# balazs-bamer/cdpr-simulation

Hardware: AMD Instinct MI355X
Metric: CDPR sim-steps/sec (whole node), 65 536 parallel 8-cable robots, 1 ms dt (higher is better)
Workload: dtype f32

## Files before the change

cdpr-simulation_amd/csrc/cdpr_engine.hip:

```cpp
#include "cdpr_engine_internal.hpp"

namespace {
thread_local std::string g_create_error;
}


namespace cdpr_host {

int derivative_weights(uint32_t n, uint32_t degree, double* w) {
  if (n < 2 || n > CDPR_MAX_D_BUFFER || degree < 1 || degree > CDPR_MAX_D_DEGREE || degree >= n) return CDPR_ERR_INVALID;
  const int m = (int)degree + 1;
  long double a[5][10];
  for (int i = 0; i < m; ++i)
    for (int j = 0; j < 2 * m; ++j) a[i][j] = 0.0L;
  std::vector<long double> x(n);
  for (uint32_t j = 0; j < n; ++j) x[j] = (long double)j - (long double)(n - 1) / 2.0L;
  for (int i = 0; i < m; ++i) {
    for (int k = 0; k < m; ++k) {
      long double s = 0;
      for (uint32_t j = 0; j < n; ++j) s += powl(x[j], i + k);
      a[i][k] = s;
    }
    a[i][m + i] = 1.0L;
  }
// ... 274 lines not shown
    case KernelId::PhysStep: return pick_phys_kernel(n, h->plan.fk, h->plan.td, kPhysStep);
    case KernelId::Rollout: return pick_rollout_kernel(n, h->plan.fk, h->plan.td);
    case KernelId::PhysRollout: return pick_phys_kernel(n, h->plan.fk, h->plan.td, kPhysRollout);
    case KernelId::PrSingle: return pick_pr_kernel(true, false, false, n, h->plan.fk, h->plan.td);
    case KernelId::PrLowreg: return pick_pr_kernel(true, false, true, n, h->plan.fk, h->plan.td);
    case KernelId::PrSplit: return pick_pr_split_kernel(n);
    case KernelId::PrMulti: return pick_pr_kernel(false, false, false, n, h->plan.fk, h->plan.td);
    case KernelId::PrRollout: return pick_pr_kernel(false, true, false, n, h->plan.fk, h->plan.td);
    case KernelId::PairSingle: return pick_pair_kernel(true, n, h->plan.fk, h->plan.td);
    case KernelId::PairMulti: return pick_pair_kernel(false, n, h->plan.fk, h->plan.td);
    case KernelId::PairStream: return pick_pair_stream_kernel(n, h->mode == kModeVelocity);
    case KernelId::Cable: return pick_cable_kernel(n, h->plan.fk, h->plan.td);
    default: return nullptr;
  }
}
StepKernel select_step_kernel(const cdpr_engine* h, int k, bool steady) { return step_kernel_of(h, planned_kernel(h->plan, launch_shape(h, k, steady))); }
bool pair_stream_steady(const cdpr_engine* h, const StepArgs& a) {
  return h->step != 0 && h->mode != kModeForce && a.pid_calls >= a.nbuf && h->cfg.publish_period == 0.0 && !a.dbg && !a.travel_on &&
         !(a.vel_limit > 0.f) && !a.unilateral && a.effort >= 0.f && a.clamp_cmd && !h->sched_ready;
}
bool split_steady_launch(const cdpr_engine* h, const PlannedKernel& pk, const StepArgs& a) {
  return pk.id == KernelId::Split && h->split_steady && !h->plan.per_robot && h->step != 0 && h->mode != kModeForce && a.pid_calls != 0 &&
         a.pid_calls >= a.nbuf && h->cfg.publish_period == 0.0 && !a.dbg && !a.travel_on;
}
uint32_t step_block_threads(const cdpr_engine* h, int k) { return planned_kernel(h->plan, launch_shape(h, k)).block; }

static int build_general(cdpr_engine* h) {
  const cdpr_config_t& cfg = h->cfg;
  h->glay.n = (int)h->n;
  h->glay.nb = (int)std::max(cfg.velocity_pid.d_buffer_length, cfg.position_pid.d_buffer_length);
  h->glay.ncas = (int)std::max(std::max(cfg.velocity_pid.p_filter.cascade, cfg.velocity_pid.d_filter.cascade),
                               std::max(cfg.position_pid.p_filter.cascade, cfg.position_pid.d_filter.cascade));
  const size_t rec_bytes = h->glay.bytes(h->stride);
  if (rec_bytes >= (1ull << 32)) {
    h->err = "general controller path: the controller records of this batch pass 4 GiB; split the batch over several handles";
    return CDPR_ERR_UNSUPPORTED;
  }
  CREATE_TRY(h, "hipMalloc(rec)", h->d_rec.alloc(rec_bytes));
  fill_gen_pid(cfg.position_pid, h->gpid[0]);
  fill_gen_pid(cfg.velocity_pid, h->gpid[1]);
  const int nbmax = h->glay.nb > 11 ? kGenMaxBuf : 11, nbp = gen_nbp(nbmax);
  std::vector<float> wt((size_t)2 * nbmax * nbp, 0.f);
  const cdpr_pid_params_t* pp[2] = {&cfg.position_pid, &cfg.velocity_pid};
  float w_new[2] = {0.f, 0.f};
  for (int p = 0; p < 2; ++p) {
    double w[CDPR_MAX_D_BUFFER];
// ... 99 lines not shown
  StepArgs a = h->base;
  a.state = st.as<float4>();
  a.obs = ob.as<float4>();
  a.cmd = cm.as<float>();
  a.dbg = nullptr;
  a.geom = h->d_geom;
  a.batch = h->plan.lane_cable ? (h->n <= 4 ? 16u : 8u) : h->plan.lane_pair ? 32u : 64u;
  a.stride = rows;
  a.nsteps = 1;
  a.obs_step_stride = 0;
  a.flags = 0u;
  a.publish_mask = 1ull;
  copy_pid(h->plan.per_robot ? h->pid_vel : h->pid_pos, a);
  copy_pid_alt(h->pid_pos, a.alt);
  a.meta = mt.as<uint8_t>();
  a.pid_calls = kCallSat;
  a.ring_slot = 0;
  set_weight_row(h, a);
  hipLaunchKernelGGL(select_step_kernel(h, 1), dim3(1), dim3(step_block_threads(h, 1)), 0, h->stream, a);
  HIP_TRY(h, hipGetLastError());
  if (planned_kernel(h->plan, launch_shape(h, 1)).id == KernelId::Split && h->split_steady) {
    for (const bool vel : {false, true}) {
      copy_pid(vel ? h->pid_vel : h->pid_pos, a);
      hipLaunchKernelGGL(pick_split_steady_kernel(h->n, vel), dim3(1), dim3(128), 0, h->stream, a);
      HIP_TRY(h, hipGetLastError());
    }
  }
  HIP_TRY(h, wait_stream(h));
  return CDPR_OK;
}

void launch_step(cdpr_engine* h, StepKernel kern, uint32_t robots_per_block, dim3 block, const StepArgs& a, uint32_t max_grid = 0) {
  const uint32_t B = a.batch;
  const uint32_t chunk = (h->plan.chunk && B > h->plan.chunk) ? h->plan.chunk : B;
  const uint32_t pieces = (B + chunk - 1u) / chunk;
  const uint32_t each = (((B + pieces - 1u) / pieces) + 63u) & ~63u;
  for (uint32_t first = 0; first < B; first += each) {
    StepArgs c = a;
    c.batch = std::min(each, B - first);
    c.state = a.state + first;
    c.obs = a.obs + first;
    if (a.cmd) c.cmd = a.cmd + (size_t)first * h->n;
    if (a.dbg) c.dbg = a.dbg + (size_t)first * CDPR_PID_DEBUG_AXES;
    if (a.meta) c.meta = a.meta + first;
    uint32_t grid = (c.batch + robots_per_block - 1u) / robots_per_block;
    if (max_grid && grid > max_grid) grid = max_grid;
    hipLaunchKernelGGL(kern, dim3(grid), block, 0, h->stream, c);
// ... 156 lines not shown
    a.cmd = h->d_target;
    a.meta = h->d_mode;
  } else {
    copy_pid(h->mode == kModeVelocity ? h->pid_vel : h->pid_pos, a);
    a.cmd = h->cmd[cmd_kind_of_mode(h->mode)].latched();
  }
  const uint32_t robots_per_block = h->plan.lane_cable ? (h->n <= 4 ? 16u : 8u) : h->plan.lane_pair ? 32u : 64u;
  const dim3 grid((h->batch + robots_per_block - 1u) / robots_per_block);

  constexpr int kGraphChunk = 10;
  int done = 0;
  while (done < nsteps) {
    const int k = std::min(per_launch, nsteps - done);
    a.nsteps = k;
    a.flags = h->plan.per_robot ? 0u : (h->mode == kModeVelocity ? kFlagActualIsVelocity : h->mode == kModeForce ? kFlagForceMode : 0u);
    const bool first_world = (h->step == 0);
    if (first_world) a.flags |= kFlagFirstWorldStep;
    a.pid_calls = sat_pid_calls(h->pid_calls);
    a.ring_slot = ring_slot_of(h->step);
    set_weight_row(h, a);
    const int kk = h->sched_refresh ? std::max(k, 2) : k;
    const PlannedKernel pk = planned_kernel(h->plan, launch_shape(h, kk, pair_stream_steady(h, a)));
    StepKernel kern = step_kernel_of(h, pk);
    h->last_variant = split_steady_launch(h, pk, a) ? 1 : 0;
    if (h->last_variant) kern = pick_split_steady_kernel(h->n, h->mode == kModeVelocity);
    const dim3 block(pk.block);
    const bool stream = pk.id == KernelId::PairStream;
    auto weights_for = [&](StepArgs& x) {
      const int slot = x.ring_slot;
      if (stream) x.ring_slot = 0;
      set_weight_row(h, x);
      x.ring_slot = slot;
    };
    if (stream) weights_for(a);
    h->last_kernel = pk;

    if (record) a.obs = record + (size_t)done * image;
    const bool steady = !record && !h->sched_refresh && h->use_graphs && (size_t)h->batch * h->n <= 131072u && !first_world && (h->plan.per_robot || a.pid_calls == kCallSat || h->mode == kModeForce) &&
                        h->cfg.publish_period == 0.0 && (nsteps - done) >= kGraphChunk * k;
    if (steady) {
      a.publish_mask = (k >= 64) ? ~0ull : ((1ull << k) - 1ull);
      cdpr_engine::GraphEntry* ge = nullptr;
      for (auto& g : h->graphs)
        if (g.kern == (void*)kern && g.cmd == a.cmd && g.steps_per_launch == k && g.flags == a.flags && g.start_slot == a.ring_slot) ge = &g;
      if (!ge) {
        cdpr_engine::GraphEntry g{(void*)kern, a.cmd, k, kGraphChunk, a.ring_slot, a.flags, nullptr, nullptr};
        bool captured = hipStreamBeginCapture(h->stream, hipStreamCaptureModeThreadLocal) == hipSuccess;
        if (captured) {
// ... 126 lines not shown
int checked(cdpr_engine* h, int rc) { return rc != CDPR_OK ? rc : check_fault(h); }

static int build_handle(cdpr_engine* h) {
  const cdpr_config_t& cfg = h->cfg;
  h->n = cfg.n_cables;
  h->batch = (uint32_t)cfg.batch;
  h->stride = (h->batch + 63u) & ~63u;
  if (h->stride % 131072u == 0u) h->stride += 128u;
  if (const char* sp = std::getenv("CDPR_STRIDE_PAD")) h->stride = ((h->batch + 63u) & ~63u) + ((uint32_t)(std::max(0L, std::atol(sp)) + 63L) & ~63u);
  h->dbg = (cfg.stages & CDPR_STAGE_PID_DEBUG) != 0;
  if (h->plan.persist) {
    h->persist_grid = (uint32_t)h->cus * 4u;
    if (const char* pg = std::getenv("CDPR_PERSIST_GRID")) h->persist_grid = (uint32_t)std::max(1L, std::atol(pg));
  }
  h->n_state = h->plan.general ? plat_slots(h->plan.fk) : state_slots((int)h->n, h->plan.fk);
  h->n_obs = obs_slots((int)h->n);
  memset(&h->base, 0, sizeof h->base);
  fill_consts(cfg, h->base);
  fill_pid(cfg.velocity_pid, cfg.dt, h->pid_vel, h->wtab_host[0]);
  fill_pid(cfg.position_pid, cfg.dt, h->pid_pos, h->wtab_host[1]);
  engine_reset_host(h);
  {
    if (const char* ss = std::getenv("CDPR_SPLIT_STEADY")) h->split_steady = !(ss[0] == '0');
    const char* ng = std::getenv("CDPR_NO_GRAPH");
    h->use_graphs = !(ng && ng[0] == '1');
  }

  CREATE_TRY(h, "hipSetDevice", hipSetDevice(h->device));
  CREATE_TRY(h, "hipStreamCreate", hipStreamCreateWithFlags(&h->stream, hipStreamNonBlocking));
  CREATE_TRY(h, "hipEventCreate", hipEventCreate(&h->ev0));
  CREATE_TRY(h, "hipEventCreate", hipEventCreate(&h->ev1));
  if (h->plan.fp64) {
    if (int rc = build_f64(h)) return rc;
  } else {
    const size_t slot_bytes = (size_t)h->stride * sizeof(float4);
    CREATE_TRY(h, "hipMalloc(state)", h->d_state.alloc(slot_bytes * h->n_state));
    CREATE_TRY(h, "hipMalloc(obs)", h->d_obs.alloc(slot_bytes * h->n_obs));
  }
  const size_t cmd_bytes = (size_t)h->stride * h->n * sizeof(float);
  for (int i = 0; i < 2; ++i)
    for (CmdChannel& c : h->cmd) {
      CREATE_TRY(h, "hipMalloc(cmd)", c.d[i].alloc(cmd_bytes));
      (void)hipMemset(c.d[i], 0, cmd_bytes);
    }
  if (int rc = upload_table(h, h->d_wtab, h->wtab_host, sizeof h->wtab_host, "wtab")) return rc;
  h->pid_vel.wtab = h->d_wtab;
// ... 610 lines not shown
  if (!h->plan.td) {
    h->err = "CDPR_STAGE_TD not enabled";
    return CDPR_ERR_UNSUPPORTED;
  }
  int rc = cdpr_get_joint_states(h, nullptr, nullptr, tension);
  if (rc != CDPR_OK) return rc;
  rc = h->plan.fp64 ? fetch_int_row64(h, kF64ObsFlags, infeasible) : fetch_fields(h, h->d_obs, {{3, 3}}, infeasible, 1u);
  if (rc == CDPR_OK && infeasible)
    for (uint32_t b = 0; b < h->batch; ++b) infeasible[b] &= 1;
  return checked(h, rc);
}

int cdpr_get_limit_state(cdpr_handle_t h, uint32_t* cable_mask) {
  if (!h || !cable_mask) return CDPR_ERR_INVALID;
  if (set_device(h) != CDPR_OK) return CDPR_ERR_DEVICE;
  int rc = h->plan.fp64 ? fetch_int_row64(h, kF64ObsFlags, reinterpret_cast<int32_t*>(cable_mask)) : fetch_fields(h, h->d_obs, {{3, 3}}, cable_mask, 1u);
  if (rc == CDPR_OK)
    for (uint32_t b = 0; b < h->batch; ++b) cable_mask[b] >>= 1;
  return checked(h, rc);
}

int cdpr_debug_last_variant(cdpr_handle_t h) { return h ? h->last_variant : -1; }

#ifdef CDPR_STAMPS
int cdpr_debug_set_stamps(cdpr_handle_t h, unsigned long long* d_stamps) {
  if (!h) return CDPR_ERR_INVALID;
  h->base.stamps = d_stamps;
  return CDPR_OK;
}
#endif

int cdpr_device_malloc(cdpr_handle_t h, size_t bytes, void** out) {
  if (!h || !out) return CDPR_ERR_INVALID;
  if (set_device(h) != CDPR_OK) return CDPR_ERR_DEVICE;
  HIP_TRY(h, hipMalloc(out, bytes));
  return CDPR_OK;
}

int cdpr_device_free(cdpr_handle_t h, void* ptr) {
  if (!h) return CDPR_ERR_INVALID;
  if (set_device(h) != CDPR_OK) return CDPR_ERR_DEVICE;
  HIP_TRY(h, hipFree(ptr));
  return CDPR_OK;
}

int cdpr_device_upload(cdpr_handle_t h, void* dst, const void* src, size_t bytes) {
// ... 37 lines not shown
```

cdpr-simulation_amd/csrc/cdpr_engine_internal.hpp:

```cpp
#pragma once
#include <hip/hip_runtime.h>

#include <atomic>
#include <chrono>

#include <algorithm>
#include <cmath>
#include <cstdio>
#include <cstring>
#include <cstdlib>
#include <string>
#include <vector>

#include "../../include/cdpr.h"
#include "cdpr_kernels.hpp"
#include "cdpr_select.hpp"
#include "cdpr_latch.hpp"
#include "cdpr_solvers.hpp"

using namespace cdpr;

namespace cdpr_host {

enum Mode { kModeForce = 0, kModePosition = 1, kModeVelocity = 2 };
// ... 118 lines not shown
  DevBuf<float> d_rec;
  DevBuf<float> d_gwtab;
  DevBuf<float> d_gptab;
  GenPid gpid[2]{};
  GenLayout glay{};
  DevBuf<double> d_roll64, d_roll64_acc;
  DevBuf<float> d_roll64_cmd;
  DevBuf<uint8_t> d_roll64_meta;
  size_t roll64_cols = 0;
  DevBuf<float> d_roll_rec;
  size_t roll_rec_cols = 0;
  struct GraphEntry {
    void* kern;
    const float* cmd;
    int steps_per_launch, launches, start_slot;
    uint32_t flags;
    hipGraph_t graph;
    hipGraphExec_t exec;
  };
  std::vector<GraphEntry> graphs;
  PlannedKernel last_kernel;
  int last_variant = 0;
  bool split_steady = true;
  int cus = 256;
  bool use_graphs = true;
  CmdChannel cmd[kCmdKinds];
  DevBuf<uint8_t> d_mode;
  DevBuf<float> d_target;
  hipStream_t copy_stream = nullptr;
  int mode = kModePosition;
  uint64_t step = 0;
  double prev_publish = 0.0;
  StepArgs base{};
  StepArgs pid_vel{}, pid_pos{};
  DevBuf<float> d_wtab;
  float wtab_host[2][kWin * (kWin + 2)]{};
  hipEvent_t ev0 = nullptr, ev1 = nullptr;
  uint64_t launches = 0, launches_mark = 0;
  PinnedBuf<float> h_pub;
  PinnedBuf<uint64_t> h_pub_done;
  DevBuf<uint32_t> d_pub_arrivals;
  uint64_t pub_epoch = 0;
  DevBuf<float> d_roll_ref;
  DevBuf<float> d_roll_cost;
  uint64_t roll_pending = 0;
  DevBuf<char> d_reset_args;
// ... 126 lines not shown
```

cdpr-simulation_amd/csrc/cdpr_kernels.hpp:

```cpp
#pragma once
#include "cdpr_step_kernel.hpp"
#include "cdpr_step_kernel_f64.hpp"
#include "cdpr_general_step.hpp"

namespace cdpr {

using StepKernel = void (*)(const StepArgs);
using F64Kernel = void (*)(const F64Args);
using GenKernel = void (*)(const StepArgs, const GenCtl);

#define CDPR_PICK_STAGES(N, EXPR)                 \
  do {                                            \
    if constexpr ((N) >= 6) {                     \
      if (fk && td) return EXPR(N, true, true);   \
      if (fk) return EXPR(N, true, false);        \
      if (td) return EXPR(N, false, true);        \
    }                                             \
    return EXPR(N, false, false);                 \
  } while (0)
#define CDPR_PICK_CABLES(FN, ...)          \
  switch (n) {                             \
    case 1: return FN<1>(__VA_ARGS__);     \
    case 2: return FN<2>(__VA_ARGS__);     \
    case 3: return FN<3>(__VA_ARGS__);     \
// ... 3 lines not shown
    case 7: return FN<7>(__VA_ARGS__);     \
    case 8: return FN<8>(__VA_ARGS__);     \
  }                                        \
  return nullptr

#define CDPR_PICK_CABLES12(FN, ...)        \
  switch (n) {                             \
    case 9: return FN<9>(__VA_ARGS__);     \
    case 10: return FN<10>(__VA_ARGS__);   \
    case 11: return FN<11>(__VA_ARGS__);   \
    case 12: return FN<12>(__VA_ARGS__);   \
  }                                        \
  CDPR_PICK_CABLES(FN, __VA_ARGS__)

StepKernel pick_step_kernel(bool single, uint32_t n, bool fk, bool td);
StepKernel pick_lowreg_kernel(uint32_t n, bool td);
StepKernel pick_rollout_kernel(uint32_t n, bool fk, bool td);
enum PhysKind { kPhysStep, kPhysRollout };
StepKernel pick_phys_kernel(uint32_t n, bool fk, bool td, int kind);
StepKernel pick_pr_kernel(bool single, bool rollout, bool lowreg, uint32_t n, bool fk, bool td);
StepKernel pick_onestep_kernel(uint32_t n, bool fk, bool td);
StepKernel pick_onestep_persist_kernel(uint32_t n, bool fk, bool td);
StepKernel pick_split_kernel(uint32_t n);
StepKernel pick_split_steady_kernel(uint32_t n, bool vel);
StepKernel pick_pr_split_kernel(uint32_t n);
StepKernel pick_pair_kernel(bool single, uint32_t n, bool fk, bool td);
StepKernel pick_pair_stream_kernel(uint32_t n, bool vel);
StepKernel pick_cable_kernel(uint32_t n, bool fk, bool td);
GenKernel pick_gen_kernel(uint32_t n, bool fk, bool td, bool rollout, bool long_window, bool single);
GenKernel pick_gen_lean11(uint32_t n);
GenKernel pick_gen_split11(uint32_t n);
F64Kernel pick_f64_split_kernel(uint32_t n, bool lean);
F64Kernel pick_f64_hold_pr_kernel(uint32_t n, bool full);
F64Kernel pick_f64_hold_long_kernel(uint32_t n, bool pr, bool tstop);
F64Kernel pick_f64_tstop_kernel(uint32_t n, bool pr = false, int hold = 0);
F64Kernel pick_f64_long_kernel(uint32_t n, bool pr = false, bool tstop = false);
F64Kernel pick_f64_split_hold_kernel(uint32_t n, bool lean, bool full);
F64Kernel pick_f64_pr_kernel(uint32_t n, bool ring_lds);
F64Kernel pick_f64_hold_kernel(uint32_t n, bool full);
F64Kernel pick_f64_kernel(uint32_t n, bool ring_lds, bool jcache);

}
```

cdpr-simulation_amd/csrc/cdpr_onestep_kernel.hpp:

```cpp
#pragma once
#include "cdpr_step_kernel.hpp"

namespace cdpr {

CDPR_DEV void row_to_lds(const float4* src, float4* dst_row) {
  __builtin_amdgcn_global_load_lds((const __attribute__((address_space(1))) void*)src, (__attribute__((address_space(3))) void*)dst_row, 16, 0, 0);
}


template <int NP, bool PR = false, bool FULL = false>
CDPR_DEV void pid_pairs(const StepArgs& a, int calls, bool is_vel, const v2f (&desired)[NP], const v2f (&actual)[NP], const v2f (&win)[NP][kWin],
                        v2f (&ierr)[NP], v2f (&f)[NP], v2f (&e_new)[NP], float& dbg_p, float& dbg_i, float& dbg_d, bool is_force = false) {
  const PidCoef c = pid_coef<PR>(a, is_vel);
  const bool run = (!PR || calls != 0) && !is_force;
  const bool full = FULL || calls >= c.nbuf;
  const float (&wt)[kWin + 2] = a.wrow;
  v2f error[NP], acc[NP];
#pragma unroll
  for (int k = 0; k < NP; ++k) {
    error[k] = desired[k] - actual[k];
    acc[k] = splat(wt[kWin]) * error[k];
  }
#pragma unroll
  for (int j = 0; j < kWin; ++j) {
// ... 364 lines not shown
  p3 = make_float4(n3.x, n3.y, n3.z, n3.w), p4 = make_float4(n4.x, n4.y, n4.z, n4.w);
  staged = run_pid;
  }
}

#ifndef CDPR_CTL_LOAD_DELAY
#define CDPR_CTL_LOAD_DELAY 8
#endif
#ifndef CDPR_SPLIT_PRIO
#define CDPR_SPLIT_PRIO 1
#endif
#ifdef CDPR_STAMPS
#define CDPR_SPLIT_STAMP(i)                                                                                          \
  do {                                                                                                               \
    __builtin_amdgcn_sched_barrier(0);                                                                               \
    if (a.stamps && lane == 0) a.stamps[(size_t)blockIdx.x * 8 + (i)] = __builtin_amdgcn_s_memrealtime();           \
    __builtin_amdgcn_sched_barrier(0);                                                                               \
  } while (0)
#else
#define CDPR_SPLIT_STAMP(i) do { } while (0)
#endif
#if defined(CDPR_STAMPS) && defined(CDPR_STAMPS_ITER)
#define CDPR_CTL_STAMP(i) do { } while (0)
#else
#define CDPR_CTL_STAMP(i) CDPR_SPLIT_STAMP(i)
#endif

template <int N, int XS, int ES, bool RAISED = true>
CDPR_DEV void split_estimator_wave(const StepArgs& a, float* geo, float gval, uint32_t lane, bool live, size_t st, uint32_t off, uint32_t woff,
                                   const float4& p0, const float4& p1, const float4& p3, const v2f* x_force, v2f* x_tension, float* x_est) {
  constexpr int NP = cable_pairs(N);
#if defined(CDPR_STAMPS) && defined(CDPR_STAMPS_CLOCK)
  const unsigned long long clk0 = __builtin_amdgcn_s_memtime();
#endif
#if CDPR_SPLIT_PRIO == 1 || CDPR_SPLIT_PRIO == 4
  if (RAISED) __builtin_amdgcn_s_setprio(3);
#elif CDPR_SPLIT_PRIO == 3 || CDPR_SPLIT_PRIO == 5
  if (RAISED) __builtin_amdgcn_s_setprio(2);
#endif
  const float4 p4 = load_slot(a.state, st, 4, off);
  if (lane < NP * kGeomFloatsPerPair) geo[lane] = gval;
  __builtin_amdgcn_fence(__ATOMIC_RELEASE, "wavefront");
  __builtin_amdgcn_wave_barrier();
  __builtin_amdgcn_fence(__ATOMIC_ACQUIRE, "wavefront");
  float fkx = p3.y, fky = p3.z, fkz = p3.w, fkqx = p4.x, fkqy = p4.y, fkqz = p4.z, fkqw = p4.w;
  v2f len[NP];
  {
    v2f jac[NP][6], l0[NP];
    ik_pairs<N, false>(geo, p0.x, p0.y, p0.z, p0.w, p1.x, p1.y, p1.z, len, jac, l0);
  }
  float fk_res = 0.f;
  int fk_it = 0;
  v2f jest[NP][6];
  {
    v2f elen[NP], unused[NP];
    bool active = true;
    for (int it = 0; it < a.fk_iters; ++it) {
      ik_pairs<N, false>(geo, fkx, fky, fkz, fkqx, fkqy, fkqz, fkqw, elen, jest, unused);
      v2f res[NP];
      v2f rm = splat(0.f);
#pragma unroll
      for (int k = 0; k < NP; ++k) {
        res[k] = len[k] - elen[k];
        rm = max2(rm, abs2(res[k]));
      }
      active = active && !(fmaxf(rm.x, rm.y) < a.fk_tol);
      float g[6];
      jt_times<NP>(jest, res, g);
      normal_solve<NP>(jest, a.fk_lambda, g);
      if (active) {
        fkx += g[0];
        fky += g[1];
        fkz += g[2];
        quat_apply_rotvec(fkqx, fkqy, fkqz, fkqw, g[3], g[4], g[5]);
        ++fk_it;
      }
#ifdef CDPR_STAMPS_ITER
      if (it < 3) {
        asm volatile("" ::"v"(fkqw));
        __builtin_amdgcn_sched_barrier(0);
        if (a.stamps && lane == 0) a.stamps[(size_t)blockIdx.x * 8 + 4 + it] = __builtin_amdgcn_s_memrealtime();
        __builtin_amdgcn_sched_barrier(0);
      }
#endif
    }
    ik_pairs<N, false>(geo, fkx, fky, fkz, fkqx, fkqy, fkqz, fkqw, elen, jest, unused);
    v2f rm = splat(0.f);
#pragma unroll
    for (int k = 0; k < NP; ++k) rm = max2(rm, abs2(len[k] - elen[k]));
    fk_res = fmaxf(rm.x, rm.y);
  }
  if (live) store_slot_aux<CDPR_SPLIT_PLAT_AUX>(a.state, st, 4, woff, make_float4(fkqx, fkqy, fkqz, fkqw));
  CDPR_SPLIT_STAMP(1);
  v2f td_l[6][3];
  float td_invd[6];
  normal_matrix_pk<NP, false>(jest, 0.f, td_l);
  chol_factor_pk(td_l, td_invd);
  __builtin_amdgcn_s_waitcnt(0xC07F);
  __builtin_amdgcn_s_barrier();
  CDPR_SPLIT_STAMP(2);
  __builtin_amdgcn_fence(__ATOMIC_ACQUIRE, "workgroup");
  v2f f[NP], df[NP], t_out[NP];
#pragma unroll
  for (int k = 0; k < NP; ++k) {
    f[k] = x_force[k * XS + lane];
    df[k] = f[k] - splat(a.td_mid);
  }
  int td_flag = 0;
// ... 9 lines not shown
      const v2f tc = max2(min2(t, splat(a.td_max)), splat(a.td_min));
      td_flag |= (tc.x != t.x) ? 1 : 0;
      if (2 * k + 1 < N) td_flag |= (tc.y != t.y) ? 1 : 0;
      t_out[k] = tc;
    }
  }
#pragma unroll
  for (int k = 0; k < NP; ++k) x_tension[k * XS + lane] = t_out[k];
  x_est[0 * ES + lane] = fkx;
  x_est[1 * ES + lane] = fky;
  x_est[2 * ES + lane] = fkz;
  x_est[3 * ES + lane] = fk_res;
  x_est[4 * ES + lane] = (float)fk_it;
  x_est[5 * ES + lane] = (float)td_flag;
  __builtin_amdgcn_fence(__ATOMIC_RELEASE, "workgroup");
  __builtin_amdgcn_s_waitcnt(0xC07F);
  CDPR_SPLIT_STAMP(3);
#if defined(CDPR_STAMPS) && defined(CDPR_STAMPS_CLOCK)
  if (a.stamps && lane == 0) a.stamps[(size_t)blockIdx.x * 8 + 7] = __builtin_amdgcn_s_memtime() - clk0;
#endif
  __builtin_amdgcn_s_barrier();
}

template <int N, bool PR, bool STEADY, bool VEL>
CDPR_DEV void split_controller_wave(const StepArgs& a, float* geo, float gval, uint32_t lane, uint32_t r, uint32_t rr, bool live, size_t st, uint32_t off,
                                    uint32_t woff, const float4& p0, const float4& p1, const float4& p2, const float4& p3, v2f* x_force, const v2f* x_tension,
                                    const float* x_est) {
  static_assert(!(STEADY && PR), "the steady instantiation serves uniform handles");
  constexpr int NP = cable_pairs(N);
  constexpr int P = plat_slots(true);
  constexpr int G = joint_groups(N);
  constexpr int NH = (NP + 1) / 2;
#if CDPR_SPLIT_PRIO == 2 || CDPR_SPLIT_PRIO == 5
  __builtin_amdgcn_s_setprio(3);
#endif
#if CDPR_CTL_LOAD_DELAY > 0
  __builtin_amdgcn_s_sleep(CDPR_CTL_LOAD_DELAY);
#endif
  float4 wraw[NP][5], hraw[NH];
#pragma unroll
  for (int k = 0; k < NP; ++k) {
#pragma unroll
    for (int m = 0; m < 5; ++m) wraw[k][m] = load_slot(a.state, st, P + 5 * k + m, off);
  }
#pragma unroll
  for (int g = 0; g < NH; ++g) hraw[g] = load_slot(a.state, st, P + 5 * NP + g, off);
  v2f desired[NP];
#pragma unroll
  for (int k = 0; k < NP; ++k) desired[k] = splat(0.f);
  const float* cp = a.cmd + (size_t)rr * N;
  if (N % 4 == 0) {
#pragma unroll
    for (int g = 0; g < N / 4; ++g) {
      const float4 v = reinterpret_cast<const float4*>(cp)[g];
      desired[2 * g] = (v2f){v.x, v.y};
      desired[2 * g + 1] = (v2f){v.z, v.w};
    }
  } else {
#pragma unroll
    for (int i = 0; i < N; ++i) {
      if (i & 1)
        desired[i / 2].y = cp[i];
      else
        desired[i / 2].x = cp[i];
    }
  }
  if (lane < NP * kGeomFloatsPerPair) geo[lane] = gval;
  __builtin_amdgcn_fence(__ATOMIC_RELEASE, "wavefront");
  __builtin_amdgcn_wave_barrier();
  __builtin_amdgcn_fence(__ATOMIC_ACQUIRE, "wavefront");

  Platform s;
  unpack_platform(p0, p1, p2, p3.x, s);

  v2f len[NP], q[NP], qd[NP], jac[NP][6];
  {
    v2f l0[NP];
    ik_pairs<N, true>(geo, s.px, s.py, s.pz, s.qx, s.qy, s.qz, s.qw, len, jac, l0);
#pragma unroll
    for (int k = 0; k < NP; ++k) {
      q[k] = l0[k] - len[k];
      qd[k] = -fma2(s.wz, jac[k][5], fma2(s.wy, jac[k][4], fma2(s.wx, jac[k][3],
                    fma2(s.vz, jac[k][2], fma2(s.vy, jac[k][1], splat(s.vx) * jac[k][0])))));
    }
  }
  const bool publish = STEADY || (a.publish_mask & 1ull) != 0ull;
  if (publish && live) {
    store_slot(a.obs, st, 0, woff, make_float4(s.px, s.py, s.pz, s.qx));
    store_slot(a.obs, st, 1, woff, make_float4(s.qy, s.qz, s.qw, s.vx));
    store_slot(a.obs, st, 2, woff, make_float4(s.vy, s.vz, s.wx, s.wy));
#pragma unroll
    for (int g = 0; g < G; ++g) {
      const int k0 = 2 * g, k1 = (2 * g + 1 < NP) ? 2 * g + 1 : 2 * g;
      const bool has = (2 * g + 1 < NP);
      store_slot(a.obs, st, 4 + g, woff, make_float4(q[k0].x, q[k0].y, has ? q[k1].x : 0.f, has ? q[k1].y : 0.f));
      store_slot(a.obs, st, 4 + G + g, woff, make_float4(qd[k0].x, qd[k0].y, has ? qd[k1].x : 0.f, has ? qd[k1].y : 0.f));
    }
  }

  v2f f[NP], e_new[NP], ierr[NP];
#pragma unroll
// ... 92 lines not shown
    for (int k = 0; k < NP; ++k) {
      tens[k] = fma2(-a.damping, qd[k], applied[k]);
      if (a.unilateral) tens[k] = max2(tens[k], splat(0.f));
    }
    float w[6];
    jt_times<NP>(jac, tens, w);
    w[0] = a.fgx - w[0];
    w[1] = a.fgy - w[1];
    w[2] = a.fgz - w[2];
    w[3] = -w[3];
    w[4] = -w[4];
    w[5] = -w[5];
    integrate(a, s, w);
  }
  if (live) {
    store_slot_aux<CDPR_SPLIT_PLAT_AUX>(a.state, st, 0, woff, make_float4(s.px, s.py, s.pz, s.qx));
    store_slot_aux<CDPR_SPLIT_PLAT_AUX>(a.state, st, 1, woff, make_float4(s.qy, s.qz, s.qw, s.vx));
    store_slot_aux<CDPR_SPLIT_PLAT_AUX>(a.state, st, 2, woff, make_float4(s.vy, s.vz, s.wx, s.wy));
    store_slot_aux<CDPR_SPLIT_PLAT_AUX>(a.state, st, 3, woff, make_float4(s.wz, fkx, fky, fkz));
  }
  CDPR_CTL_STAMP(6);
}

template <int N, bool PR, bool STEADY, bool VEL>
CDPR_DEV void split_kernel_body(const StepArgs& a) {
  constexpr int NP = cable_pairs(N);
  __shared__ __attribute__((aligned(16))) float lds[2][NP * kGeomFloatsPerPair];
  __shared__ v2f x_force[NP][64];
  __shared__ v2f x_tension[NP][64];
  __shared__ float x_est[6][64];

  const uint32_t swap = __builtin_popcount(blockIdx.x & a.split_swap) & 1u;
  const uint32_t wave = (threadIdx.x >> 6) ^ swap, lane = threadIdx.x & 63u;
  const uint32_t r = blockIdx.x * 64u + lane;
  const uint32_t rr = (r < a.batch) ? r : (a.batch - 1u);
  const bool live = r < a.batch;
  const size_t st = a.stride;
  const uint32_t off = rr * 16u, woff = r * 16u;
  float* const geo = lds[wave];

  if (wave == 0) CDPR_SPLIT_STAMP(0);
#ifdef CDPR_STAMPS
  if (a.stamps && lane == 0)
    reinterpret_cast<uint32_t*>(&a.stamps[(size_t)blockIdx.x * 8 + 7])[threadIdx.x >> 6] =
        (__builtin_amdgcn_s_getreg((16 - 1) << 11 | 4) & 0xffffu) | ((__builtin_amdgcn_s_getreg((4 - 1) << 11 | 20) & 0xfu) << 16);
#endif
  const float gval = (lane < NP * kGeomFloatsPerPair) ? a.geom[lane] : 0.f;
  const float4 p0 = load_slot(a.state, st, 0, off), p1 = load_slot(a.state, st, 1, off), p2 = load_slot(a.state, st, 2, off),
               p3 = load_slot(a.state, st, 3, off);
  if (wave == 0) {
    split_estimator_wave<N, 64, 64>(a, geo, gval, lane, live, st, off, woff, p0, p1, p3, &x_force[0][0], &x_tension[0][0], &x_est[0][0]);
    return;
  }
  split_controller_wave<N, PR, STEADY, VEL>(a, geo, gval, lane, r, rr, live, st, off, woff, p0, p1, p2, p3, &x_force[0][0], &x_tension[0][0], &x_est[0][0]);
}
template <int N, bool PR = false>
__global__ __launch_bounds__(128, 2) void cdpr_split_kernel(const StepArgs a) { split_kernel_body<N, PR, false, false>(a); }
template <int N, bool VEL>
__global__ __launch_bounds__(128, 2) void cdpr_split_steady_kernel(const StepArgs a) { split_kernel_body<N, false, true, VEL>(a); }

}
```

cdpr-simulation_amd/csrc/k_onestep.hip:

```cpp
#include "cdpr_kernels.hpp"
#include "cdpr_onestep_kernel.hpp"
namespace cdpr {
namespace {
#define K_ONE(N, FK, TD) cdpr_onestep_kernel<N, FK, TD>
#define K_ONE_PERSIST(N, FK, TD) cdpr_onestep_kernel<N, FK, TD, true>
template <int N> StepKernel one_n(bool fk, bool td) { CDPR_PICK_STAGES(N, K_ONE); }
template <int N> StepKernel one_persist_n(bool fk, bool td) { CDPR_PICK_STAGES(N, K_ONE_PERSIST); }
}
StepKernel pick_onestep_kernel(uint32_t n, bool fk, bool td) { CDPR_PICK_CABLES(one_n, fk, td); }
StepKernel pick_onestep_persist_kernel(uint32_t n, bool fk, bool td) { CDPR_PICK_CABLES(one_persist_n, fk, td); }
StepKernel pick_split_kernel(uint32_t n) {
  switch (n) {
    case 6: return cdpr_split_kernel<6>;
    case 7: return cdpr_split_kernel<7>;
    case 8: return cdpr_split_kernel<8>;
  }
  return nullptr;
}
StepKernel pick_split_steady_kernel(uint32_t n, bool vel) {
  switch (n) {
    case 6: return vel ? cdpr_split_steady_kernel<6, true> : cdpr_split_steady_kernel<6, false>;
    case 7: return vel ? cdpr_split_steady_kernel<7, true> : cdpr_split_steady_kernel<7, false>;
    case 8: return vel ? cdpr_split_steady_kernel<8, true> : cdpr_split_steady_kernel<8, false>;
  }
  return nullptr;
}
StepKernel pick_pr_split_kernel(uint32_t n) {
  switch (n) {
    case 6: return cdpr_split_kernel<6, true>;
    case 7: return cdpr_split_kernel<7, true>;
    case 8: return cdpr_split_kernel<8, true>;
  }
  return nullptr;
}
}
```

cdpr-simulation_amd/engine.py:

```python
from __future__ import annotations

import ctypes as C
from typing import Optional, Tuple

import numpy as np

from . import _abi
from ._native import lib
from .config import Config, DoneRule


class CdprError(RuntimeError):
    def __init__(self, code: int, message: str):
        super().__init__(f"cdpr error {code}: {message}")
        self.code = code


def _fp(a: Optional[np.ndarray]):
    return None if a is None else a.ctypes.data_as(C.POINTER(C.c_float))


def derivative_weights(n: int, degree: int) -> np.ndarray:
    w = np.empty(n, dtype=np.float64)
    rc = lib().cdpr_derivative_weights(n, degree, w.ctypes.data_as(C.POINTER(C.c_double)))
# ... 173 lines not shown
        return out

    def decode_observables(self, image: np.ndarray):
        img = np.ascontiguousarray(image, dtype=np.uint8)
        out = [np.empty((self.B, w), dtype=np.float32) for w in (self.n, self.n, self.n, 7, 6)]
        self._check(lib().cdpr_decode_observables(self._h, img.ctypes.data_as(C.c_void_p), *[_fp(o) for o in out]))
        return tuple(out)

    def synchronize(self) -> None:
        self._check(lib().cdpr_synchronize(self._h))

    @property
    def step_count(self) -> int:
        return int(lib().cdpr_step_count(self._h))

    @property
    def kernel_name(self) -> str:
        buf = C.create_string_buffer(256)
        self._check(lib().cdpr_kernel_name(self._h, buf, 256))
        return buf.value.decode()

    @property
    def last_variant(self) -> int:
        fn = lib().cdpr_debug_last_variant
        fn.argtypes, fn.restype = [C.c_void_p], C.c_int
        return int(fn(self._h))

    @property
    def mapping(self) -> str:
        return {_abi.MAP_LANE_PER_ROBOT: "lane-per-robot", _abi.MAP_LANE_PAIR: "lane-pair", _abi.MAP_LANE_PER_CABLE: "lane-per-cable"}.get(int(lib().cdpr_mapping(self._h)), "auto")

    @property
    def sim_time(self) -> float:
        return self.step_count * self.config.dt

    def joint_states(self) -> Tuple[np.ndarray, np.ndarray, np.ndarray]:
        q, qd, e = (np.empty((self.B, self.n), dtype=np.float32) for _ in range(3))
        self._check(lib().cdpr_get_joint_states(self._h, _fp(q), _fp(qd), _fp(e)))
        return q, qd, e

    def platform_state(self) -> Tuple[np.ndarray, np.ndarray]:
        p, t = np.empty((self.B, 7), dtype=np.float32), np.empty((self.B, 6), dtype=np.float32)
        self._check(lib().cdpr_get_platform_state(self._h, _fp(p), _fp(t)))
        return p, t

    def observables(self):
        q, qd, e = (np.empty((self.B, self.n), dtype=np.float32) for _ in range(3))
        p, t = np.empty((self.B, 7), dtype=np.float32), np.empty((self.B, 6), dtype=np.float32)
        self._check(lib().cdpr_get_observables(self._h, _fp(q), _fp(qd), _fp(e), _fp(p), _fp(t)))
# ... 156 lines not shown
```

Before: 6.432 billion.

## Add steady split-kernel estimator variants without FK tolerance test and with shared true-state IK

When FK tolerance is zero, the steady split kernel now gets specialised estimator variants. TOL0 drops the per-iteration residual max and convergence test. ONE_IK goes further: the estimator wave skips its own true-state IK and reads the cable lengths the controller wave computed and shared through LDS, then runs a reordered Newton loop that reuses the Jacobian from the previous IK evaluation. Both are enabled by default, with environment toggles and a debug hook for setting the FK estimate. The cost is an extra workgroup barrier coupling the two waves and controller loads deferred until after the barrier, which can add stalls.

```diff
diff --git a/cdpr-simulation_amd/csrc/cdpr_engine.hip b/cdpr-simulation_amd/csrc/cdpr_engine.hip
--- a/cdpr-simulation_amd/csrc/cdpr_engine.hip
+++ b/cdpr-simulation_amd/csrc/cdpr_engine.hip
@@ -320,6 +320,10 @@
 bool split_steady_launch(const cdpr_engine* h, const PlannedKernel& pk, const StepArgs& a) {
   return pk.id == KernelId::Split && h->split_steady && !h->plan.per_robot && h->step != 0 && h->mode != kModeForce && a.pid_calls != 0 &&
          a.pid_calls >= a.nbuf && h->cfg.publish_period == 0.0 && !a.dbg && !a.travel_on;
+}
+int split_steady_estimator(const cdpr_engine* h) {
+  if (!h->split_steady_est || h->cfg.fk_tolerance != 0.0) return 0;
+  return h->split_one_ik ? 2 : 1;
 }
 uint32_t step_block_threads(const cdpr_engine* h, int k) { return planned_kernel(h->plan, launch_shape(h, k)).block; }
 
@@ -465,7 +469,7 @@
   if (planned_kernel(h->plan, launch_shape(h, 1)).id == KernelId::Split && h->split_steady) {
     for (const bool vel : {false, true}) {
       copy_pid(vel ? h->pid_vel : h->pid_pos, a);
-      hipLaunchKernelGGL(pick_split_steady_kernel(h->n, vel), dim3(1), dim3(128), 0, h->stream, a);
+      hipLaunchKernelGGL(pick_split_steady_kernel(h->n, vel, split_steady_estimator(h)), dim3(1), dim3(128), 0, h->stream, a);
       HIP_TRY(h, hipGetLastError());
     }
   }
@@ -668,8 +672,12 @@
     const int kk = h->sched_refresh ? std::max(k, 2) : k;
     const PlannedKernel pk = planned_kernel(h->plan, launch_shape(h, kk, pair_stream_steady(h, a)));
     StepKernel kern = step_kernel_of(h, pk);
-    h->last_variant = split_steady_launch(h, pk, a) ? 1 : 0;
-    if (h->last_variant) kern = pick_split_steady_kernel(h->n, h->mode == kModeVelocity);
+    h->last_variant = 0;
+    if (split_steady_launch(h, pk, a)) {
+      const int est = split_steady_estimator(h);
+      h->last_variant = est == 2 ? 7 : est == 1 ? 3 : 1;
+      kern = pick_split_steady_kernel(h->n, h->mode == kModeVelocity, est);
+    }
     const dim3 block(pk.block);
     const bool stream = pk.id == KernelId::PairStream;
     auto weights_for = [&](StepArgs& x) {
@@ -842,6 +850,8 @@
   engine_reset_host(h);
   {
     if (const char* ss = std::getenv("CDPR_SPLIT_STEADY")) h->split_steady = !(ss[0] == '0');
+    if (const char* ss = std::getenv("CDPR_SPLIT_STEADY_EST")) h->split_steady_est = !(ss[0] == '0');
+    if (const char* ss = std::getenv("CDPR_SPLIT_ONE_IK")) h->split_one_ik = !(ss[0] == '0');
     const char* ng = std::getenv("CDPR_NO_GRAPH");
     h->use_graphs = !(ng && ng[0] == '1');
   }
@@ -1498,6 +1508,25 @@
 
 int cdpr_debug_last_variant(cdpr_handle_t h) { return h ? h->last_variant : -1; }
 
+int cdpr_debug_set_fk_estimate(cdpr_handle_t h, const float* pose7) {
+  if (!h || !pose7 || h->plan.fp64 || !h->plan.fk) return CDPR_ERR_INVALID;
+  if (set_device(h) != CDPR_OK) return CDPR_ERR_DEVICE;
+  const int P = plat_slots(true);
+  std::vector<float4> s;
+  const int rc = fetch_slots(h, h->d_state, P, s);
+  if (rc != CDPR_OK) return rc;
+  const size_t st = h->stride;
+  for (uint32_t r = 0; r < h->batch; ++r) {
+    const float* p = pose7 + (size_t)r * 7;
+    float4& d = s[3 * st + r];
+    d.y = p[0]; d.z = p[1]; d.w = p[2];
+    s[4 * st + r] = make_float4(p[3], p[4], p[5], p[6]);
+  }
+  HIP_TRY(h, hipMemcpyAsync(h->d_state, s.data(), s.size() * sizeof(float4), hipMemcpyHostToDevice, h->stream));
+  HIP_TRY(h, wait_stream(h));
+  return CDPR_OK;
+}
+
 #ifdef CDPR_STAMPS
 int cdpr_debug_set_stamps(cdpr_handle_t h, unsigned long long* d_stamps) {
   if (!h) return CDPR_ERR_INVALID;
diff --git a/cdpr-simulation_amd/csrc/cdpr_engine_internal.hpp b/cdpr-simulation_amd/csrc/cdpr_engine_internal.hpp
--- a/cdpr-simulation_amd/csrc/cdpr_engine_internal.hpp
+++ b/cdpr-simulation_amd/csrc/cdpr_engine_internal.hpp
@@ -164,6 +164,8 @@
   PlannedKernel last_kernel;
   int last_variant = 0;
   bool split_steady = true;
+  bool split_steady_est = true;
+  bool split_one_ik = true;
   int cus = 256;
   bool use_graphs = true;
   CmdChannel cmd[kCmdKinds];
diff --git a/cdpr-simulation_amd/csrc/cdpr_kernels.hpp b/cdpr-simulation_amd/csrc/cdpr_kernels.hpp
--- a/cdpr-simulation_amd/csrc/cdpr_kernels.hpp
+++ b/cdpr-simulation_amd/csrc/cdpr_kernels.hpp
@@ -49,7 +49,7 @@
 StepKernel pick_onestep_kernel(uint32_t n, bool fk, bool td);
 StepKernel pick_onestep_persist_kernel(uint32_t n, bool fk, bool td);
 StepKernel pick_split_kernel(uint32_t n);
-StepKernel pick_split_steady_kernel(uint32_t n, bool vel);
+StepKernel pick_split_steady_kernel(uint32_t n, bool vel, int est = 0);
 StepKernel pick_pr_split_kernel(uint32_t n);
 StepKernel pick_pair_kernel(bool single, uint32_t n, bool fk, bool td);
 StepKernel pick_pair_stream_kernel(uint32_t n, bool vel);
diff --git a/cdpr-simulation_amd/csrc/cdpr_onestep_kernel.hpp b/cdpr-simulation_amd/csrc/cdpr_onestep_kernel.hpp
--- a/cdpr-simulation_amd/csrc/cdpr_onestep_kernel.hpp
+++ b/cdpr-simulation_amd/csrc/cdpr_onestep_kernel.hpp
@@ -410,13 +410,20 @@
 #endif
 #if defined(CDPR_STAMPS) && defined(CDPR_STAMPS_ITER)
 #define CDPR_CTL_STAMP(i) do { } while (0)
+#define CDPR_IK0_STAMP(i) do { } while (0)
+#elif defined(CDPR_STAMPS) && defined(CDPR_STAMPS_IK0)
+#define CDPR_CTL_STAMP(i) do { } while (0)
+#define CDPR_IK0_STAMP(i) CDPR_SPLIT_STAMP(i)
 #else
 #define CDPR_CTL_STAMP(i) CDPR_SPLIT_STAMP(i)
-#endif
-
-template <int N, int XS, int ES, bool RAISED = true>
+#define CDPR_IK0_STAMP(i) do { } while (0)
+#endif
+
+template <int N, int XS, int ES, bool RAISED = true, bool TOL0 = false, bool ONE_IK = false>
 CDPR_DEV void split_estimator_wave(const StepArgs& a, float* geo, float gval, uint32_t lane, bool live, size_t st, uint32_t off, uint32_t woff,
-                                   const float4& p0, const float4& p1, const float4& p3, const v2f* x_force, v2f* x_tension, float* x_est) {
+                                   const float4& p0, const float4& p1, const float4& p3, const v2f* x_force, v2f* x_tension, float* x_est,
+                                   const v2f* x_len = nullptr) {
+  static_assert(!ONE_IK || TOL0, "the rotated Newton loop has no convergence test");
   constexpr int NP = cable_pairs(N);
 #if defined(CDPR_STAMPS) && defined(CDPR_STAMPS_CLOCK)
   const unsigned long long clk0 = __builtin_amdgcn_s_memtime();
@@ -433,14 +440,44 @@
   __builtin_amdgcn_fence(__ATOMIC_ACQUIRE, "wavefront");
   float fkx = p3.y, fky = p3.z, fkz = p3.w, fkqx = p4.x, fkqy = p4.y, fkqz = p4.z, fkqw = p4.w;
   v2f len[NP];
-  {
+  if (!ONE_IK) {
     v2f jac[NP][6], l0[NP];
     ik_pairs<N, false>(geo, p0.x, p0.y, p0.z, p0.w, p1.x, p1.y, p1.z, len, jac, l0);
   }
   float fk_res = 0.f;
   int fk_it = 0;
   v2f jest[NP][6];
-  {
+  if (ONE_IK) {
+    v2f elen[NP], unused[NP];
+    ik_pairs<N, false>(geo, fkx, fky, fkz, fkqx, fkqy, fkqz, fkqw, elen, jest, unused);
+#pragma unroll
+    for (int k = 0; k < NP; ++k) asm volatile("" : "+v"(elen[k]), "+v"(jest[k][0]), "+v"(jest[k][1]), "+v"(jest[k][2]), "+v"(jest[k][3]), "+v"(jest[k][4]), "+v"(jest[k][5]));
+    __builtin_amdgcn_s_waitcnt(0xC07F);
+    CDPR_IK0_STAMP(4);
+    __builtin_amdgcn_s_barrier();
+    CDPR_IK0_STAMP(5);
+    __builtin_amdgcn_fence(__ATOMIC_ACQUIRE, "workgroup");
+#pragma unroll
+    for (int k = 0; k < NP; ++k) len[k] = x_len[k * XS + lane];
+    for (int it = 0; it < a.fk_iters; ++it) {
+      v2f res[NP];
+#pragma unroll
+      for (int k = 0; k < NP; ++k) res[k] = len[k] - elen[k];
+      float g[6];
+      jt_times<NP>(jest, res, g);
+      normal_solve<NP>(jest, a.fk_lambda, g);
+      fkx += g[0];
+      fky += g[1];
+      fkz += g[2];
+      quat_apply_rotvec(fkqx, fkqy, fkqz, fkqw, g[3], g[4], g[5]);
+      ik_pairs<N, false>(geo, fkx, fky, fkz, fkqx, fkqy, fkqz, fkqw, elen, jest, unused);
+    }
+    fk_it = max(a.fk_iters, 0);
+    v2f rm = splat(0.f);
+#pragma unroll
+    for (int k = 0; k < NP; ++k) rm = max2(rm, abs2(len[k] - elen[k]));
+    fk_res = fmaxf(rm.x, rm.y);
+  } else {
     v2f elen[NP], unused[NP];
     bool active = true;
     for (int it = 0; it < a.fk_iters; ++it) {
@@ -450,18 +487,18 @@
 #pragma unroll
       for (int k = 0; k < NP; ++k) {
         res[k] = len[k] - elen[k];
-        rm = max2(rm, abs2(res[k]));
-      }
-      active = active && !(fmaxf(rm.x, rm.y) < a.fk_tol);
+        if (!TOL0) rm = max2(rm, abs2(res[k]));
+      }
+      if (!TOL0) active = active && !(fmaxf(rm.x, rm.y) < a.fk_tol);
       float g[6];
       jt_times<NP>(jest, res, g);
       normal_solve<NP>(jest, a.fk_lambda, g);
-      if (active) {
+      if (TOL0 || active) {
         fkx += g[0];
         fky += g[1];
         fkz += g[2];
         quat_apply_rotvec(fkqx, fkqy, fkqz, fkqw, g[3], g[4], g[5]);
-        ++fk_it;
+        if (!TOL0) ++fk_it;
       }
 #ifdef CDPR_STAMPS_ITER
       if (it < 3) {
@@ -472,6 +509,7 @@
       }
 #endif
     }
+    if (TOL0) fk_it = max(a.fk_iters, 0);
     ik_pairs<N, false>(geo, fkx, fky, fkz, fkqx, fkqy, fkqz, fkqw, elen, jest, unused);
     v2f rm = splat(0.f);
 #pragma unroll
@@ -527,11 +565,37 @@
   __builtin_amdgcn_s_barrier();
 }
 
-template <int N, bool PR, bool STEADY, bool VEL>
+template <int N>
+CDPR_DEV void load_desired(const float* cp, v2f (&desired)[cable_pairs(N)]) {
+#pragma unroll
+  for (int k = 0; k < cable_pairs(N); ++k) desired[k] = splat(0.f);
+  if (N % 4 == 0) {
+#pragma unroll
+    for (int g = 0; g < N / 4; ++g) {
+      const float4 v = reinterpret_cast<const float4*>(cp)[g];
+      desired[2 * g] = (v2f){v.x, v.y};
+      desired[2 * g + 1] = (v2f){v.z, v.w};
+    }
+  } else {
+#pragma unroll
+    for (int i = 0; i < N; ++i) {
+      if (i & 1)
+        desired[i / 2].y = cp[i];
+      else
+        desired[i / 2].x = cp[i];
+    }
+  }
+}
+
+#ifndef CDPR_ONE_IK_PRIO
+#define CDPR_ONE_IK_PRIO 0
+#endif
+template <int N, bool PR, bool STEADY, bool VEL, bool ONE_IK = false>
 CDPR_DEV void split_controller_wave(const StepArgs& a, float* geo, float gval, uint32_t lane, uint32_t r, uint32_t rr, bool live, size_t st, uint32_t off,
                                     uint32_t woff, const float4& p0, const float4& p1, const float4& p2, const float4& p3, v2f* x_force, const v2f* x_tension,
-                                    const float* x_est) {
+                                    const float* x_est, v2f* x_len = nullptr) {
   static_assert(!(STEADY && PR), "the steady instantiation serves uniform handles");
+  static_assert(!ONE_IK || STEADY, "one true-state IK: the steady kernel only");
   constexpr int NP = cable_pairs(N);
   constexpr int P = plat_slots(true);
   constexpr int G = joint_groups(N);
@@ -539,37 +603,25 @@
 #if CDPR_SPLIT_PRIO == 2 || CDPR_SPLIT_PRIO == 5
   __builtin_amdgcn_s_setprio(3);
 #endif
+#if CDPR_ONE_IK_PRIO == 1
+  if (ONE_IK) __builtin_amdgcn_s_setprio(3);
+#endif
 #if CDPR_CTL_LOAD_DELAY > 0
-  __builtin_amdgcn_s_sleep(CDPR_CTL_LOAD_DELAY);
+  if (!ONE_IK) __builtin_amdgcn_s_sleep(CDPR_CTL_LOAD_DELAY);
 #endif
   float4 wraw[NP][5], hraw[NH];
-#pragma unroll
-  for (int k = 0; k < NP; ++k) {
-#pragma unroll
-    for (int m = 0; m < 5; ++m) wraw[k][m] = load_slot(a.state, st, P + 5 * k + m, off);
-  }
-#pragma unroll
-  for (int g = 0; g < NH; ++g) hraw[g] = load_slot(a.state, st, P + 5 * NP + g, off);
   v2f desired[NP];
-#pragma unroll
-  for (int k = 0; k < NP; ++k) desired[k] = splat(0.f);
+  if (!ONE_IK) {
+#pragma unroll
+    for (int k = 0; k < NP; ++k) {
+#pragma unroll
+      for (int m = 0; m < 5; ++m) wraw[k][m] = load_slot(a.state, st, P + 5 * k + m, off);
+    }
+#pragma unroll
+    for (int g = 0; g < NH; ++g) hraw[g] = load_slot(a.state, st, P + 5 * NP + g, off);
+  }
   const float* cp = a.cmd + (size_t)rr * N;
-  if (N % 4 == 0) {
-#pragma unroll
-    for (int g = 0; g < N / 4; ++g) {
-      const float4 v = reinterpret_cast<const float4*>(cp)[g];
-      desired[2 * g] = (v2f){v.x, v.y};
-      desired[2 * g + 1] = (v2f){v.z, v.w};
-    }
-  } else {
-#pragma unroll
-    for (int i = 0; i < N; ++i) {
-      if (i & 1)
-        desired[i / 2].y = cp[i];
-      else
-        desired[i / 2].x = cp[i];
-    }
-  }
+  if (!ONE_IK) load_desired<N>(cp, desired);
   if (lane < NP * kGeomFloatsPerPair) geo[lane] = gval;
   __builtin_amdgcn_fence(__ATOMIC_RELEASE, "wavefront");
   __builtin_amdgcn_wave_barrier();
@@ -582,6 +634,24 @@
   {
     v2f l0[NP];
     ik_pairs<N, true>(geo, s.px, s.py, s.pz, s.qx, s.qy, s.qz, s.qw, len, jac, l0);
+    if (ONE_IK) {
+#pragma unroll
+      for (int k = 0; k < NP; ++k) x_len[k * 64 + lane] = len[k];
+      __builtin_amdgcn_fence(__ATOMIC_RELEASE, "workgroup");
+      __builtin_amdgcn_s_waitcnt(0xC07F);
+#if CDPR_ONE_IK_PRIO == 1
+      __builtin_amdgcn_s_setprio(0);
+#endif
+      __builtin_amdgcn_s_barrier();
+#pragma unroll
+      for (int k = 0; k < NP; ++k) {
+#pragma unroll
+        for (int m = 0; m < 5; ++m) wraw[k][m] = load_slot(a.state, st, P + 5 * k + m, off);
+      }
+#pragma unroll
+      for (int g = 0; g < NH; ++g) hraw[g] = load_slot(a.state, st, P + 5 * NP + g, off);
+      load_desired<N>(cp, desired);
+    }
 #pragma unroll
     for (int k = 0; k < NP; ++k) {
       q[k] = l0[k] - len[k];
@@ -720,13 +790,14 @@
   CDPR_CTL_STAMP(6);
 }
 
-template <int N, bool PR, bool STEADY, bool VEL>
+template <int N, bool PR, bool STEADY, bool VEL, bool TOL0 = false, bool ONE_IK = false>
 CDPR_DEV void split_kernel_body(const StepArgs& a) {
   constexpr int NP = cable_pairs(N);
   __shared__ __attribute__((aligned(16))) float lds[2][NP * kGeomFloatsPerPair];
   __shared__ v2f x_force[NP][64];
   __shared__ v2f x_tension[NP][64];
   __shared__ float x_est[6][64];
+  __shared__ v2f x_len[ONE_IK ? NP : 1][64];
 
   const uint32_t swap = __builtin_popcount(blockIdx.x & a.split_swap) & 1u;
   const uint32_t wave = (threadIdx.x >> 6) ^ swap, lane = threadIdx.x & 63u;
@@ -747,14 +818,16 @@
   const float4 p0 = load_slot(a.state, st, 0, off), p1 = load_slot(a.state, st, 1, off), p2 = load_slot(a.state, st, 2, off),
                p3 = load_slot(a.state, st, 3, off);
   if (wave == 0) {
-    split_estimator_wave<N, 64, 64>(a, geo, gval, lane, live, st, off, woff, p0, p1, p3, &x_force[0][0], &x_tension[0][0], &x_est[0][0]);
+    split_estimator_wave<N, 64, 64, true, TOL0, ONE_IK>(a, geo, gval, lane, live, st, off, woff, p0, p1, p3, &x_force[0][0], &x_tension[0][0], &x_est[0][0],
+                                                        ONE_IK ? &x_len[0][0] : nullptr);
     return;
   }
-  split_controller_wave<N, PR, STEADY, VEL>(a, geo, gval, lane, r, rr, live, st, off, woff, p0, p1, p2, p3, &x_force[0][0], &x_tension[0][0], &x_est[0][0]);
+  split_controller_wave<N, PR, STEADY, VEL, ONE_IK>(a, geo, gval, lane, r, rr, live, st, off, woff, p0, p1, p2, p3, &x_force[0][0], &x_tension[0][0], &x_est[0][0],
+                                                    ONE_IK ? &x_len[0][0] : nullptr);
 }
 template <int N, bool PR = false>
 __global__ __launch_bounds__(128, 2) void cdpr_split_kernel(const StepArgs a) { split_kernel_body<N, PR, false, false>(a); }
-template <int N, bool VEL>
-__global__ __launch_bounds__(128, 2) void cdpr_split_steady_kernel(const StepArgs a) { split_kernel_body<N, false, true, VEL>(a); }
+template <int N, bool VEL, bool TOL0 = false, bool ONE_IK = false>
+__global__ __launch_bounds__(128, 2) void cdpr_split_steady_kernel(const StepArgs a) { split_kernel_body<N, false, true, VEL, TOL0, ONE_IK>(a); }
 
 }
diff --git a/cdpr-simulation_amd/csrc/k_onestep.hip b/cdpr-simulation_amd/csrc/k_onestep.hip
--- a/cdpr-simulation_amd/csrc/k_onestep.hip
+++ b/cdpr-simulation_amd/csrc/k_onestep.hip
@@ -17,11 +17,18 @@
   }
   return nullptr;
 }
-StepKernel pick_split_steady_kernel(uint32_t n, bool vel) {
+namespace {
+template <int N> StepKernel split_steady_n(bool vel, int est) {
+  if (est == 2) return vel ? cdpr_split_steady_kernel<N, true, true, true> : cdpr_split_steady_kernel<N, false, true, true>;
+  if (est == 1) return vel ? cdpr_split_steady_kernel<N, true, true> : cdpr_split_steady_kernel<N, false, true>;
+  return vel ? cdpr_split_steady_kernel<N, true> : cdpr_split_steady_kernel<N, false>;
+}
+}
+StepKernel pick_split_steady_kernel(uint32_t n, bool vel, int est) {
   switch (n) {
-    case 6: return vel ? cdpr_split_steady_kernel<6, true> : cdpr_split_steady_kernel<6, false>;
-    case 7: return vel ? cdpr_split_steady_kernel<7, true> : cdpr_split_steady_kernel<7, false>;
-    case 8: return vel ? cdpr_split_steady_kernel<8, true> : cdpr_split_steady_kernel<8, false>;
+    case 6: return split_steady_n<6>(vel, est);
+    case 7: return split_steady_n<7>(vel, est);
+    case 8: return split_steady_n<8>(vel, est);
   }
   return nullptr;
 }
diff --git a/cdpr-simulation_amd/engine.py b/cdpr-simulation_amd/engine.py
--- a/cdpr-simulation_amd/engine.py
+++ b/cdpr-simulation_amd/engine.py
@@ -219,9 +219,18 @@
 
     @property
     def last_variant(self) -> int:
+        return self.last_variant_word & 1
+
+    @property
+    def last_variant_word(self) -> int:
         fn = lib().cdpr_debug_last_variant
         fn.argtypes, fn.restype = [C.c_void_p], C.c_int
         return int(fn(self._h))
+
+    def debug_set_fk_estimate(self, pose7) -> None:
+        fn = lib().cdpr_debug_set_fk_estimate
+        fn.argtypes, fn.restype = [C.c_void_p, C.POINTER(C.c_float)], C.c_int
+        self._check(fn(self._h, _fp(np.ascontiguousarray(pose7, dtype=np.float32).reshape(self.B, 7))))
 
     @property
     def mapping(self) -> str:
```

After: 6.356 billion. 0.988x the previous value.
